# FunAudioLLM/CosyVoice

Measured on NVIDIA H100. Metric: audio-sec/s, CosyVoice2-0.5B zero-shot batch-32, NFE=10, higher is better.
Workload: dtype bf16

## Files before the change

### cosyvoice_b200/csrc/api.cu

```cuda
#include "common.cuh"
#include <string.h>
#include <algorithm>

void hift_build(cvk_ctx* ctx);
void hift_f0(cvk_ctx* ctx, const float* mel, const int* lens, int B, float* f0_out, cudaStream_t st);
void hift_source(cvk_ctx* ctx, const float* f0, const int* lens, int B, const float* noise, float* source_out, cudaStream_t st);
void hift_decode(cvk_ctx* ctx, const float* mel, const int* lens, int B, const float* source, float* wav, cudaStream_t st);
void hift_inference(cvk_ctx* ctx, const float* mel, const int* lens, int B, const float* noise, const float* cache_source,
                    const int* cache_lens, float* wav, float* source_out, cudaStream_t st);
void flow_build(cvk_ctx* ctx, const int* cfg, int ncfg);
void flow_encoder(cvk_ctx* ctx, const int32_t* tokens, const int* lens, int B, int streaming, int context_len, float* h, cudaStream_t st);
void flow_estimator(cvk_ctx* ctx, const float* x, const float* mu, const float* t, const float* spks, const float* cond, const int* lens,
                    int B, int streaming, float* out, cudaStream_t st);
void flow_cfm_solve(cvk_ctx* ctx, const float* mu, const float* spks, const float* cond, const int* lens, int B, const float* z,
                    int n_timesteps, float cfg_rate, int streaming, float* out, cudaStream_t st);
void flow_inference(cvk_ctx* ctx, const int32_t* tokens, const int* token_lens, const float* prompt_feat, const int* prompt_feat_lens,
                    const float* embedding, int B, int n_timesteps, int streaming, int finalize, float* mel, cudaStream_t st);
void flow_set_noise(cvk_ctx* ctx, const float* noise_tm, int T, int on_device);
void llm_build(cvk_ctx* ctx, const int* cfg, int ncfg);
cvk_lm_session* llm_session_create(cvk_ctx* ctx, int max_batch, int max_context);
void llm_session_destroy(cvk_ctx* ctx, cvk_lm_session* s);
void hift3_build(cvk_ctx* ctx);
void hift3_set_noise(cvk_ctx* ctx, const float* rand_ini, const float* sine_noise, long long n, int on_device);
void hift3_inference(cvk_ctx* ctx, const float* mel, const int* lens, const int* finalize, int B, float* wav, float* f0_out,
// ... 22 lines not shown
                    const float* uniforms, const int32_t* ignore_eos, int32_t* out_ids, cudaStream_t st);
void llm_decode_attention_op(cvk_ctx* ctx, const float* partial, int splits, int rows, const float* bias, float* k_cache, float* v_cache,
                             const int* ctx_len_host, int max_ctx, float* out, cudaStream_t st);
void llm_decode_layers_op(cvk_ctx* ctx, int B, const int* ctx_len_host, int max_ctx, float* x, float* k_cache, float* v_cache,
                          float* xn_out, float* att_out, float* ffa_out, cudaStream_t st);
void llm_sample_step_op(cvk_ctx* ctx, float* logits, int B, int V, const float* uniforms, const int32_t* min_len, const int32_t* max_len,
                        int32_t* out_ids, int out_ld, int32_t* out_count, int32_t* done, int* ctx_len, const int* base_len, int* live,
                        const float* speech_emb, float* next_x, const float* gamma, float* xn, cudaStream_t st);
void llm_log_softmax_op(cvk_ctx* ctx, float* x, int rows, int V, cudaStream_t st);
void mel_spectrogram(cvk_ctx* ctx, const float* wav, const int* lens, int B, int fmax_hz, float* mel, cudaStream_t st);
void mel_init(cvk_ctx* ctx);
void mel_resample(cvk_ctx* ctx, const float* mel, const int* lens, const int* out_lens, int B, float* out, cudaStream_t st);
void prompt_feat_init(cvk_ctx* ctx);

#define CVK_API_BEGIN            \
  if (!ctx) return CVK_ERR_INVALID; \
  try {                          \
    cudaSetDevice(ctx->device);
#define CVK_API_END                                  \
    return CVK_OK;                                   \
  } catch (const CvkError& e) {                      \
    ctx->last_error = e.what();                      \
    return e.code;                                   \
  } catch (const std::exception& e) {                \
    ctx->last_error = std::string("internal: ") + e.what(); \
    return CVK_ERR_INVALID;                          \
  }

typedef CUresult (*EncodeTiledFn)(CUtensorMap*, CUtensorMapDataType, cuuint32_t, void*, const cuuint64_t*, const cuuint64_t*,
                                  const cuuint32_t*, const cuuint32_t*, CUtensorMapInterleave, CUtensorMapSwizzle,
                                  CUtensorMapL2promotion, CUtensorMapFloatOOBfill);

void encode_tma_map(cvk_ctx* ctx, CUtensorMap* map, const void* base, int rank, const cuuint64_t* dims, const cuuint64_t* strides,
                    const cuuint32_t* box, int dtype, CUtensorMapL2promotion l2, const char* what) {
  CVK_REQUIRE(rank == 2 || rank == 3, std::string("tensor map ") + what + ": rank 2 or 3");
  const cuuint32_t es[3] = {1, 1, 1};
  CUresult r = ((EncodeTiledFn)ctx->encode_tiled)(map, dtype == DT_F32 ? CU_TENSOR_MAP_DATA_TYPE_FLOAT32 : CU_TENSOR_MAP_DATA_TYPE_BFLOAT16, rank,
                                                  const_cast<void*>(base), dims, strides, box, es, CU_TENSOR_MAP_INTERLEAVE_NONE,
                                                  CU_TENSOR_MAP_SWIZZLE_128B, l2, CU_TENSOR_MAP_FLOAT_OOB_FILL_NONE);
  CVK_REQUIRE(r == CUDA_SUCCESS, std::string("cuTensorMapEncodeTiled(") + what + ") failed: " + std::to_string((int)r));
}

extern "C" {

const char* cvk_version(void) { return "libcvk 0.1 (sm_90a)"; }

int cvk_create(int device, int precision, size_t workspace_bytes, cvk_ctx** out) {
  if (!out) return CVK_ERR_INVALID;
  *out = nullptr;
  int n = 0;
  if (cudaGetDeviceCount(&n) != cudaSuccess || n <= device || device < 0) return CVK_ERR_CUDA;
  if (precision != CVK_PREC_FP32 && precision != CVK_PREC_BF16) return CVK_ERR_INVALID;
  if (cudaSetDevice(device) != cudaSuccess) return CVK_ERR_CUDA;
  cudaDeviceProp prop;
  if (cudaGetDeviceProperties(&prop, device) != cudaSuccess) return CVK_ERR_CUDA;
  if (prop.major != 9) return CVK_ERR_CUDA;
  void* encode = nullptr;
  cudaDriverEntryPointQueryResult qres;
  if (cudaGetDriverEntryPoint("cuTensorMapEncodeTiled", &encode, cudaEnableDefault, &qres) != cudaSuccess ||
      qres != cudaDriverEntryPointSuccess || !encode)
    return CVK_ERR_CUDA;
  try {
    gemm_tc_setup();
    attention_tc_setup();
    skinny_setup();
    hift3_setup();
  } catch (const std::exception&) {
    return CVK_ERR_CUDA;
  }
  cvk_ctx* ctx = new cvk_ctx();
  ctx->device = device;
  ctx->precision = precision;
// ... 22 lines not shown
  delete ctx;
}

const char* cvk_last_error(cvk_ctx* ctx) { return ctx ? ctx->last_error.c_str() : "null context"; }
thread_local int cvk_in_capture = 0;
int64_t cvk_launch_count(cvk_ctx* ctx) { return ctx ? ctx->launches.load() : 0; }
int cvk_stream_create(cvk_ctx* ctx, void** out) {
  CVK_API_BEGIN
  CVK_REQUIRE(out != nullptr, "cvk_stream_create: bad arguments");
  cudaStream_t s = nullptr;
  CVK_CHECK_CUDA(cudaStreamCreateWithFlags(&s, cudaStreamNonBlocking));
  *out = (void*)s;
  CVK_API_END
}
void cvk_stream_destroy(cvk_ctx* ctx, void* stream) {
  if (!ctx || !stream) return;
  cudaSetDevice(ctx->device);
  cudaStreamDestroy((cudaStream_t)stream);
}
double cvk_last_op_ms(cvk_ctx* ctx) { return ctx ? ctx->op_ms : 0.0; }
int cvk_debug_read(cvk_ctx* ctx, long long* out, int n) {
  if (!ctx || !ctx->tl || !out || n != 4096) return CVK_ERR_INVALID;
  cudaSetDevice(ctx->device);
  if (cudaMemcpy(out, ctx->tl, 4096 * sizeof(long long), cudaMemcpyDeviceToHost) != cudaSuccess) return CVK_ERR_CUDA;
  return CVK_OK;
}

int cvk_set_option(cvk_ctx* ctx, const char* key, int value) {
  CVK_API_BEGIN
  std::string k(key ? key : "");
  if (k == "use_tc") ctx->use_tc = value;
  else if (k == "flow_fused_ff") ctx->flow_fused_ff = value;
  else if (k == "flow_qkv_panel") ctx->flow_qkv_panel = value;
  else if (k == "tc_epi") ctx->tc_epi = value;
  else if (k == "tc_persist") ctx->tc_persist = value;
  else if (k == "op_out_bf16") ctx->op_out_bf16 = value;
  else if (k == "op_iters") ctx->op_iters = value;
  else if (k == "use_graph") ctx->use_graph = value;
  else if (k == "use_tc_attn") ctx->use_tc_attn = value;
  else if (k == "use_skinny") ctx->use_skinny = value;
  else if (k == "lm_fused") ctx->lm_fused = value;
  else if (k == "pdl") ctx->pdl = value;
  else if (k == "lm_mega") ctx->lm_mega = value;
  else if (k == "enc_tc_attn") ctx->enc_tc_attn = value;
  else if (k == "hift_f16") ctx->hift_f16 = value;
  else if (k == "mega_coop") ctx->mega_coop = value;
  else if (k == "chain_timeline") {
    if (value && !ctx->tl) {
      ctx->tl = ctx->dmalloc(4096 * sizeof(long long));
      CVK_CHECK_CUDA(cudaMemset(ctx->tl, 0, 4096 * sizeof(long long)));
    }
    if (!value) ctx->tl = nullptr;
  }
  else throw CvkError(CVK_ERR_INVALID, "unknown option: " + k);
  CVK_API_END
}

int cvk_profile(cvk_ctx* ctx, int enable) {
  CVK_API_BEGIN
  CVK_CHECK_CUDA(cudaDeviceSynchronize());
  for (auto& r : ctx->prof) { ctx->event_pool.push_back(r.a); ctx->event_pool.push_back(r.b); }
  ctx->prof.clear();
  ctx->prof_on = enable;
  CVK_API_END
}

// ... 697 lines not shown
```

### cosyvoice_b200/csrc/cvk_internal.h

```cpp
#pragma once
#include <cuda_runtime.h>
#include <cuda_bf16.h>
#include <cuda_fp16.h>
#include <cuda.h>
#include <stdint.h>
#include <stdio.h>
#include <string>
#include <vector>
#include <map>
#include <unordered_map>
#include <stdexcept>
#include <atomic>

#include "../../include/cvk.h"

typedef __nv_bfloat16 bf16;

struct CvkError : std::runtime_error {
  int code;
  CvkError(int c, const std::string& m) : std::runtime_error(m), code(c) {}
};

#define CVK_CHECK_CUDA(expr)                                                                       \
  do {                                                                                             \
// ... 124 lines not shown
  void* prompt_feat_model = nullptr;
  void* encode_tiled = nullptr;
  std::atomic<int64_t> launches{0};
  int op_out_bf16 = 0;
  int op_iters = 0;
  double op_ms = 0.0;
  int tc_epi = 2;
  int tc_persist = 2;
  void* tl = nullptr;
  int tl_seq = 0;
  long long* tl_next() {
    if (!tl) return nullptr;
    long long* p = (long long*)tl + 4 * (tl_seq % 1024);
    ++tl_seq;
    return p;
  }
  int prof_on = 0;
  std::vector<ProfRec> prof;
  std::unordered_map<const void*, void*> tiled;
  std::vector<cudaEvent_t> event_pool;
  int pdl = 1;
  int lm_fused = 1;
  int hift_f16 = 1;
  int build_f16 = 0;
  int enc_tc_attn = 1;
  int lm_mega = 0;
  int mega_coop = 1;
  int use_skinny = 1;
  int use_tc_attn = 1;
  int use_graph = 1;
  int use_tc = 1;
  int flow_fused_ff = 1;
  int flow_qkv_panel = 1;

  void* dmalloc(size_t bytes) {
    void* p = nullptr;
    CVK_CHECK_CUDA(cudaMalloc(&p, bytes ? bytes : 16));
    owned.push_back(p);
    return p;
  }
  const RawTensor& get_raw(const std::string& name) const {
    auto it = raw.find(name);
    if (it == raw.end()) throw CvkError(CVK_ERR_MISSING_WEIGHT, "missing weight tensor: " + name);
    return it->second;
  }
  bool has_raw(const std::string& name) const { return raw.find(name) != raw.end(); }
};

template <typename... KArgs, typename... Args>
inline void launch_ex(void (*kern)(KArgs...), dim3 grid, dim3 block, size_t smem, cudaStream_t st, bool pdl, Args&&... args) {
  cudaLaunchConfig_t cfg = {};
  cfg.gridDim = grid;
  cfg.blockDim = block;
  cfg.dynamicSmemBytes = smem;
  cfg.stream = st;
  cudaLaunchAttribute at[1];
  if (pdl) {
    at[0].id = cudaLaunchAttributeProgrammaticStreamSerialization;
    at[0].val.programmaticStreamSerializationAllowed = 1;
    cfg.attrs = at;
    cfg.numAttrs = 1;
  }
  CVK_CHECK_CUDA(cudaLaunchKernelEx(&cfg, kern, KArgs(std::forward<Args>(args))...));
}

void encode_tma_map(cvk_ctx* ctx, CUtensorMap* map, const void* base, int rank, const cuuint64_t* dims, const cuuint64_t* strides,
                    const cuuint32_t* box, int dtype, CUtensorMapL2promotion l2, const char* what);
void gemm_tc_setup();
void attention_tc_setup();
void skinny_setup();
void hift3_setup();

Seqs make_seqs(cvk_ctx* ctx, const int* lens, int B, int gap, int scale, int extra_front, cudaStream_t st, bool with_row2seq = true);
Seqs scale_seqs(cvk_ctx* ctx, const Seqs& s, int scale, int extra_front, cudaStream_t st, bool with_row2seq = true);

ConvW make_linear(cvk_ctx* ctx, const std::string& wname, const std::string& bname);
ConvW make_conv(cvk_ctx* ctx, const float* w_oik , const float* bias, int N, int K, int taps,
                int dil, int shift0);
ConvW make_conv_named(cvk_ctx* ctx, const std::string& wname, const std::string& bname, int dil, int shift0);
float* fold_weight_norm(cvk_ctx* ctx, const std::string& prefix, int64_t* numel_out);
void finish_convw(cvk_ctx* ctx, ConvW& w);
float* dev_copy_f32(cvk_ctx* ctx, const float* src_dev, size_t n);

void conv_gemm(cvk_ctx* ctx, cudaStream_t st, const Mat& A, const ConvW& W, const Epilogue& ep);
void conv_gemm_simt(cvk_ctx* ctx, cudaStream_t st, const Mat& A, const ConvW& W, const Epilogue& ep);
void conv_gemm_tc(cvk_ctx* ctx, cudaStream_t st, const Mat& A, const ConvW& W, const Epilogue& ep);
void ffn_fused(cvk_ctx* ctx, cudaStream_t st, const Mat& x, const int* row2seq, const float* ln3_g, const float* ln3_b, const ConvW& w1,
               const ConvW& w2, const float* ln_g, const float* ln_b, const Mat& out);
void flow_ff(cvk_ctx* ctx, cudaStream_t st, const Mat& x, const int* row2seq, const float* ln3_g, const float* ln3_b, const ConvW& ff1,
             const ConvW& ff2, const float* ln_g, const float* ln_b, const Mat& out, const Mat& xn, const Mat& hid);
size_t skinny_scratch_floats(int rows, int maxN);
const bf16* skinny_tiled_weights(cvk_ctx* ctx, const ConvW& W);
int conv_gemm_skinny_ex(cvk_ctx* ctx, cudaStream_t st, const Mat& A, const ConvW& W, const Epilogue& ep, float* scratch, size_t scratch_floats,
                        int mode);
void conv_gemm_skinny(cvk_ctx* ctx, cudaStream_t st, const Mat& A, const ConvW& W, const Epilogue& ep, float* scratch, size_t scratch_floats);

void zero_mat(cvk_ctx* ctx, cudaStream_t st, const Mat& m);
void layernorm(cvk_ctx* ctx, cudaStream_t st, const Mat& x, const float* gamma, const float* beta, float eps, int act,
               float post_scale, const int* row2seq, const Mat& out, const float* rowvec = nullptr, int rowvec_ld = 0);
void unpack_rows_skip(cvk_ctx* ctx, cudaStream_t st, const Mat& in, const Seqs& s, const int* skip_host, float* dense, int C);
Seqs shrink_seqs(cvk_ctx* ctx, const Seqs& s, int drop_tail, cudaStream_t st);
Seqs shrink_seqs(cvk_ctx* ctx, const Seqs& s, const int* drop_tail_host , cudaStream_t st);
Seqs subseqs(cvk_ctx* ctx, const Seqs& s, const int* skip_host, cudaStream_t st);
void rmsnorm(cvk_ctx* ctx, cudaStream_t st, const Mat& x, const float* gamma, float eps, const Mat& out);
void act_copy(cvk_ctx* ctx, cudaStream_t st, const Mat& x, int act, float param, const float* alpha, const int* row2seq,
              const Mat& out);
void act_copy_scaled(cvk_ctx* ctx, cudaStream_t st, const Mat& x, float pre_scale, int act, float param, const float* alpha,
                     const int* row2seq, const Mat& out);
void pack_rows(cvk_ctx* ctx, cudaStream_t st, const float* dense, int C, const Seqs& s, const Mat& out);
void unpack_rows(cvk_ctx* ctx, cudaStream_t st, const Mat& in, const Seqs& s, int skip, float* dense, int C);
void bcast_rows(cvk_ctx* ctx, cudaStream_t st, const float* vec, int C, int vec_ld, const Seqs& s, const Mat& out);
void convert_mat(cvk_ctx* ctx, cudaStream_t st, const Mat& in, const Mat& out);

struct KvGeom {
  const int* d_kstart = nullptr;
  const int* d_klen = nullptr;
  const int* d_qoff = nullptr;
};
void whisper_log_mel(cvk_ctx* ctx, const float* wav, const int* lens, int B, float* out, cudaStream_t st);
void kaldi_fbank80(cvk_ctx* ctx, const float* wav, const int* lens, int B, int subtract_mean, float* out, cudaStream_t st);
struct cvk_flow_stream;
// ... 46 lines not shown
```

### cosyvoice_b200/csrc/gemm_tc.cu

```cuda
#include "common.cuh"
#include "wgmma.cuh"
#include "tma.cuh"

namespace {

constexpr int TC_BM = 128;
constexpr int TC_BK = 64;
constexpr int TC_THREADS = 384;

__device__ __forceinline__ void epi_store16(const EpiDev& e, int r, int n0, int N, const float* acc) {
  if (n0 + 16 > N) {
    for (int i = 0; i < 16 && n0 + i < N; ++i) epi_store<true>(e, r, n0 + i, acc[i]);
    return;
  }
  int seq = 0;
  bool valid = true;
  if (e.row2seq) {
    seq = e.row2seq[r];
    valid = seq >= 0;
  }
  float v[16];
#pragma unroll
  for (int i = 0; i < 16; ++i) v[i] = acc[i];
  if (e.bias) {
// ... 156 lines not shown
    const float* rv = e.rowvec + (size_t)seq * e.rowvec_ld + n0;
#pragma unroll
    for (int i = 0; i < 16; i += 4) {
      const float4 b = *reinterpret_cast<const float4*>(rv + i);
      v[i] += b.x; v[i + 1] += b.y; v[i + 2] += b.z; v[i + 3] += b.w;
    }
  }
  act16_fast(e.act1, v, e.act1_param, e.alpha1 ? e.alpha1 + n0 : nullptr);
#pragma unroll
  for (int i = 0; i < 16; ++i) v[i] *= e.scale;
  if (e.resid && rin) {
    const float* rp = e.resid + (size_t)r * e.resid_ld + n0;
#pragma unroll
    for (int i = 0; i < 16; i += 4) {
      const float4 b = *reinterpret_cast<const float4*>(rp + i);
      v[i] += b.x; v[i + 1] += b.y; v[i + 2] += b.z; v[i + 3] += b.w;
    }
  }
  if (!valid) {
#pragma unroll
    for (int i = 0; i < 16; ++i) v[i] = 0.f;
  }
  if (e.out2) {
#pragma unroll
    for (int i = 0; i < 16; ++i) w2[i] = v[i];
    act16_fast(e.act2, w2, e.act2_param, e.alpha2 ? e.alpha2 + n0 : nullptr);
    if (!valid) {
#pragma unroll
      for (int i = 0; i < 16; ++i) w2[i] = 0.f;
    }
  }
}

__device__ __forceinline__ void stage_store16(uint32_t stg, int dtype, int row, int c, const float* v) {
  if (dtype != DT_F32) {
    const uint32_t sub = stg + (uint32_t)(c >> 6) * 16384u + (uint32_t)row * 128u;
    const uint32_t ch = (uint32_t)((c & 63) >> 3);
    uint32_t pk[8];
    if (dtype == DT_BF16) {
#pragma unroll
      for (int i = 0; i < 16; i += 2) {
        __nv_bfloat162 h2 = __floats2bfloat162_rn(v[i], v[i + 1]);
        pk[i >> 1] = *reinterpret_cast<uint32_t*>(&h2);
      }
    } else {
#pragma unroll
      for (int i = 0; i < 16; i += 2) pk[i >> 1] = (uint32_t)f32_to_16(v[i], DT_F16) | ((uint32_t)f32_to_16(v[i + 1], DT_F16) << 16);
    }
    asm volatile("st.shared.v4.b32 [%0], {%1,%2,%3,%4};" ::"r"(sub + ((ch ^ (uint32_t)(row & 7)) << 4)), "r"(pk[0]), "r"(pk[1]), "r"(pk[2]), "r"(pk[3]) : "memory");
    asm volatile("st.shared.v4.b32 [%0], {%1,%2,%3,%4};" ::"r"(sub + (((ch + 1) ^ (uint32_t)(row & 7)) << 4)), "r"(pk[4]), "r"(pk[5]), "r"(pk[6]), "r"(pk[7]) : "memory");
  } else {
    const uint32_t sub = stg + (uint32_t)(c >> 5) * 16384u + (uint32_t)row * 128u;
    const uint32_t ch = (uint32_t)((c & 31) >> 2);
#pragma unroll
    for (int j = 0; j < 4; ++j) {
      asm volatile("st.shared.v4.b32 [%0], {%1,%2,%3,%4};" ::"r"(sub + (((ch + j) ^ (uint32_t)(row & 7)) << 4)), "r"(__float_as_uint(v[4 * j])),
                   "r"(__float_as_uint(v[4 * j + 1])), "r"(__float_as_uint(v[4 * j + 2])), "r"(__float_as_uint(v[4 * j + 3]))
                   : "memory");
    }
  }
}

constexpr uint32_t TC_STG_BYTES = 65536;

template <int BN, int NSTG>
__global__ void __launch_bounds__(TC_THREADS, 1)
conv_gemm_wg_kernel(const __grid_constant__ CUtensorMap tmap_a, const __grid_constant__ CUtensorMap tmap_w,
                    const __grid_constant__ CUtensorMap tmap_o, const __grid_constant__ CUtensorMap tmap_o2, int N, int K, int taps,
                    int dil, int shift0, int rowsOut, EpiDev ep, int epi_mode, int ntn, int ntiles) {
  extern __shared__ uint8_t smem_raw[];
  __shared__ __align__(8) uint64_t bar_full[NSTG];
  __shared__ __align__(8) uint64_t bar_empty[NSTG];
  __shared__ __align__(16) float s_bias[BN];
  constexpr uint32_t A_BYTES = TC_BM * TC_BK * 2;
  constexpr uint32_t B_BYTES = BN * TC_BK * 2;
  constexpr uint32_t STAGE_BYTES = A_BYTES + B_BYTES;
  const uint32_t smem_base = (smem_u32(smem_raw) + 1023u) & ~1023u;
  const uint32_t stg_base = smem_base + NSTG * STAGE_BYTES;
  const int warp = threadIdx.x >> 5, lane = threadIdx.x & 31;
  const int kchunks = (K + TC_BK - 1) / TC_BK;
  const int iters = taps * kchunks;

  if (threadIdx.x == 0) {
    for (int s = 0; s < NSTG; ++s) {
      mbar_init(smem_u32(&bar_full[s]), 1);
      mbar_init(smem_u32(&bar_empty[s]), 8);
    }
    asm volatile("fence.mbarrier_init.release.cluster;" ::: "memory");
  }
  __syncthreads();

  if (warp < 4) {
    if (warp == 0 && lane == 0) {
// ... 421 lines not shown
    const int rb = wg * 64 + (warp & 3) * 16 + (lane >> 2);
#pragma unroll
    for (int j = 0; j < 32; ++j) {
      const int col = 8 * j + 2 * q;
      const float2 b = *reinterpret_cast<const float2*>(p.b2 + col);
      *reinterpret_cast<float2*>(stg + rb * FF_OLD + col) = make_float2(o[4 * j] + b.x, o[4 * j + 1] + b.y);
      *reinterpret_cast<float2*>(stg + (rb + 8) * FF_OLD + col) = make_float2(o[4 * j + 2] + b.x, o[4 * j + 3] + b.y);
    }
  }
  asm volatile("bar.sync 1, 256;" ::: "memory");

  for (int i = 0; i < 16; ++i) {
    const int row = cw * 16 + i, r = r0 + row;
    if (r >= p.rows) break;
    const bool valid = p.row2seq[r] >= 0;
    float* xp = p.x + (size_t)r * p.ldx;
    const float* sp = stg + row * FF_OLD;
    const float4 sa = *reinterpret_cast<const float4*>(sp + c0), sb = *reinterpret_cast<const float4*>(sp + c1);
    const float4 xa = *reinterpret_cast<const float4*>(xp + c0), xb = *reinterpret_cast<const float4*>(xp + c1);
    float v[8] = {sa.x + xa.x, sa.y + xa.y, sa.z + xa.z, sa.w + xa.w, sb.x + xb.x, sb.y + xb.y, sb.z + xb.z, sb.w + xb.w};
    if (!valid) {
#pragma unroll
      for (int j = 0; j < 8; ++j) v[j] = 0.f;
    }
    *reinterpret_cast<float4*>(xp + c0) = make_float4(v[0], v[1], v[2], v[3]);
    *reinterpret_cast<float4*>(xp + c1) = make_float4(v[4], v[5], v[6], v[7]);
    if (p.ln_g && valid) ln256_warp(v, p.ln_g, p.ln_b, 1e-5f, c0, c1);
    bf16* op = p.out + (size_t)r * p.ldo;
    __nv_bfloat162 h0 = __floats2bfloat162_rn(v[0], v[1]), h1 = __floats2bfloat162_rn(v[2], v[3]);
    __nv_bfloat162 h2 = __floats2bfloat162_rn(v[4], v[5]), h3 = __floats2bfloat162_rn(v[6], v[7]);
    *reinterpret_cast<uint2*>(op + c0) = make_uint2(*reinterpret_cast<uint32_t*>(&h0), *reinterpret_cast<uint32_t*>(&h1));
    *reinterpret_cast<uint2*>(op + c1) = make_uint2(*reinterpret_cast<uint32_t*>(&h2), *reinterpret_cast<uint32_t*>(&h3));
  }
}

}

void conv_gemm_tc(cvk_ctx* ctx, cudaStream_t st, const Mat& A, const ConvW& W, const Epilogue& ep) {
  CVK_REQUIRE((A.dtype == DT_BF16 && W.w16 != nullptr) || (A.dtype == DT_F16 && W.wf16 != nullptr), "conv_gemm_tc: 16-bit operands (A and W of the same kind) required");
  const void* w16p = A.dtype == DT_F16 ? (const void*)W.wf16 : (const void*)W.w16;
  CVK_REQUIRE(A.cols >= W.K, "conv_gemm_tc: A has fewer columns than K");
  CVK_REQUIRE(W.K % 8 == 0 && A.ld % 8 == 0 && ((uintptr_t)A.p & 15) == 0, "conv_gemm_tc: operands must be 16-byte aligned");
  CVK_REQUIRE(ep.out.p != nullptr && ep.out.cols >= W.N, "conv_gemm_tc: bad output");
  const int BN = W.N > 64 ? 128 : 64;
  CUtensorMap ta, tw;
  {
    const cuuint64_t dims[2] = {(cuuint64_t)W.K, (cuuint64_t)A.rows};
    const cuuint64_t strides[1] = {(cuuint64_t)A.ld * 2};
    const cuuint32_t box[2] = {TC_BK, TC_BM};
    encode_tma_map(ctx, &ta, A.p, 2, dims, strides, box, A.dtype, CU_TENSOR_MAP_L2_PROMOTION_L2_128B, "A");
  }
  {
    const cuuint64_t dims[3] = {(cuuint64_t)W.K, (cuuint64_t)W.taps, (cuuint64_t)W.N};
    const cuuint64_t strides[2] = {(cuuint64_t)W.K * 2, (cuuint64_t)W.K * W.taps * 2};
    const cuuint32_t box[3] = {TC_BK, 1, (cuuint32_t)BN};
    encode_tma_map(ctx, &tw, w16p, 3, dims, strides, box, A.dtype, CU_TENSOR_MAP_L2_PROMOTION_L2_256B, "W");
  }
  EpiDev e = to_dev(ep);
  e.ab_f16 = A.dtype == DT_F16;
  if (!e.bias) e.bias = W.bias;
  int rowsOut = ep.out.rows;
  CVK_REQUIRE((ep.out.ld * ep.out.esize()) % 16 == 0 && ((uintptr_t)ep.out.p & 15) == 0, "conv_gemm_tc: output rows must be 16-byte aligned");
  CVK_REQUIRE(!ep.resid.p || (ep.resid.ld % 4 == 0 && ((uintptr_t)ep.resid.p & 15) == 0), "conv_gemm_tc: residual alignment");
  CVK_REQUIRE(!(ep.resid.p && ep.rowvec), "conv_gemm_tc: residual and per-sequence vector cannot be combined");
  CVK_REQUIRE(!ep.rowvec || (ep.rowvec_ld % 4 == 0 && ((uintptr_t)ep.rowvec & 15) == 0), "conv_gemm_tc: rowvec alignment");
  CVK_REQUIRE(!ep.out2.p || ((ep.out2.ld * ep.out2.esize()) % 16 == 0 && ((uintptr_t)ep.out2.p & 15) == 0), "conv_gemm_tc: out2 alignment");
// ... 27 lines not shown
}

void ffn_fused(cvk_ctx* ctx, cudaStream_t st, const Mat& x, const int* row2seq, const float* ln3_g, const float* ln3_b, const ConvW& w1,
               const ConvW& w2, const float* ln_g, const float* ln_b, const Mat& out) {
  CVK_REQUIRE(x.dtype == DT_F32 && x.cols == FF_C && x.ld % 4 == 0 && ((uintptr_t)x.p & 15) == 0, "ffn_fused: x must be fp32 [rows, 256], 16-byte aligned rows");
  CVK_REQUIRE(out.dtype == DT_BF16 && out.cols == FF_C && out.rows >= x.rows && out.ld % 8 == 0 && ((uintptr_t)out.p & 15) == 0,
              "ffn_fused: out must be bf16 [rows, 256], 16-byte aligned rows");
  CVK_REQUIRE(w1.N == FF_HID && w1.K == FF_C && w1.taps == 1 && w1.w16 && w1.bias && w2.N == FF_C && w2.K == FF_HID && w2.taps == 1 && w2.w16 &&
                  w2.bias && row2seq && ln3_g && ln3_b && (!ln_g || ln_b),
              "ffn_fused: unexpected weights");
  CVK_REQUIRE((((uintptr_t)ln3_g | (uintptr_t)ln3_b | (uintptr_t)ln_g | (uintptr_t)ln_b | (uintptr_t)w1.bias | (uintptr_t)w2.bias) & 15) == 0,
              "ffn_fused: LayerNorm and bias vectors must be 16-byte aligned");
  CUtensorMap t1, t2;
  auto mk = [&](CUtensorMap* m, const bf16* w, int N, int K, int box_n) {
    const cuuint64_t dims[2] = {(cuuint64_t)K, (cuuint64_t)N};
    const cuuint64_t strides[1] = {(cuuint64_t)K * 2};
    const cuuint32_t box[2] = {64, (cuuint32_t)box_n};
    encode_tma_map(ctx, m, w, 2, dims, strides, box, DT_BF16, CU_TENSOR_MAP_L2_PROMOTION_L2_256B, "ffn weights");
  };
  mk(&t1, w1.w16, FF_HID, FF_C, FF_HC);
  mk(&t2, w2.w16, FF_C, FF_HID, FF_C);
  FfnDev p;
  p.x = x.f32(); p.ldx = x.ld; p.rows = x.rows; p.row2seq = row2seq;
  p.ln3_g = ln3_g; p.ln3_b = ln3_b; p.b1 = w1.bias; p.b2 = w2.bias; p.ln_g = ln_g; p.ln_b = ln_b;
  p.out = out.b16(); p.ldo = out.ld;
  const double flops = 4.0 * x.rows * (double)FF_C * FF_HID;
  const double bytes = (double)x.rows * FF_C * (4 + 4 + 2) + 2.0 * FF_C * FF_HID * 2;
  ProfScope ps(ctx, st, FAM_GEMM_TC, flops, bytes);
  ffn_fused_kernel<<<ceil_div(x.rows, TC_BM), TC_THREADS, FF_SMEM, st>>>(t1, t2, p);
  ctx->launches++;
  CVK_LAUNCH_CHECK();
}

void gemm_tc_setup() {
  CVK_CHECK_CUDA(cudaFuncSetAttribute(conv_gemm_wg_kernel<128, 4>, cudaFuncAttributeMaxDynamicSharedMemorySize, (int)wg_smem<128, 4>()));
  CVK_CHECK_CUDA(cudaFuncSetAttribute(conv_gemm_wg_kernel<64, 4>, cudaFuncAttributeMaxDynamicSharedMemorySize, (int)wg_smem<64, 4>()));
  CVK_CHECK_CUDA(cudaFuncSetAttribute(qkv_panel_kernel, cudaFuncAttributeMaxDynamicSharedMemorySize, (int)QP_SMEM));
  CVK_CHECK_CUDA(cudaFuncSetAttribute(ffn_fused_kernel, cudaFuncAttributeMaxDynamicSharedMemorySize, (int)FF_SMEM));
}
```

### cosyvoice_b200/csrc/hift.cu

```cuda
#include "common.cuh"

namespace {

constexpr int kUps[3] = {8, 5, 3};
constexpr int kUpK[3] = {16, 11, 7};
constexpr int kRbK[3] = {3, 7, 11};
constexpr int kSrcRbK[3] = {7, 7, 11};
constexpr int kDil[3] = {1, 3, 5};
constexpr int kCh[4] = {512, 256, 128, 64};
constexpr int kUpscale = 480;
constexpr int kStftLd = 24;

struct ResBlockW {
  ConvW c1[3], c2[3];
  float* a1[3];
  float* a2[3];
};

}

struct HiftModel {
  bool half_weights = false;
  ConvW f0_conv[5];
  ConvW f0_cls;
// ... 336 lines not shown

static int* upload_ints(cvk_ctx* ctx, const std::vector<int>& v, cudaStream_t st) {
  int* d = (int*)ctx->arena.alloc(sizeof(int) * v.size());
  CVK_CHECK_CUDA(cudaMemcpyAsync(d, v.data(), sizeof(int) * v.size(), cudaMemcpyHostToDevice, st));
  return d;
}

static std::vector<int> prefix_offsets(const int* lens, int B) {
  std::vector<int> off(B);
  int acc = 0;
  for (int b = 0; b < B; ++b) { off[b] = acc; acc += lens[b]; }
  return off;
}

static void hift_source_packed(cvk_ctx* ctx, cudaStream_t st, const Seqs& s0, const int* lens, const Mat& f0, const float* noise,
                               float* src_packed) {
  HiftModel* m = ctx->hift;
  float* phase = (float*)ctx->arena.alloc(sizeof(float) * 9 * (size_t)s0.R);
  phase_kernel<<<s0.B, 32, 0, st>>>(f0.f32(), f0.ld, s0.d_start, s0.d_len, phase);
  ctx->launches++;
  CVK_LAUNCH_CHECK();
  CVK_CHECK_CUDA(cudaMemsetAsync(src_packed, 0, sizeof(float) * (size_t)s0.R * kUpscale, st));
  int* noff = upload_ints(ctx, prefix_offsets(lens, s0.B), st);
  int bx = ceil_div(s0.max_len * kUpscale, 256);
  if (bx > 512) bx = 512;
  source_kernel<<<dim3(bx, s0.B), 256, 0, st>>>(f0.f32(), f0.ld, phase, s0.d_start, s0.d_len, noise, noff, m->src_w, m->src_b, src_packed);
  ctx->launches++;
  CVK_LAUNCH_CHECK();
}

static void run_resblock(cvk_ctx* ctx, cudaStream_t st, const ResBlockW& rb, const Seqs& s, const Mat& x ,
                         const Mat& a , const Mat& ya, const Mat& xr ,
                         const Mat& final_out, int final_accumulate) {
  for (int d = 0; d < 3; ++d) {
    Epilogue e1;
    e1.act1 = ACT_SNAKE;
    e1.alpha1 = rb.a2[d];
    e1.row2seq = s.d_row2seq;
    e1.out = ya;
    conv_gemm(ctx, st, a, rb.c1[d], e1);
    Epilogue e2;
    e2.resid = d == 0 ? x : xr;
    e2.row2seq = s.d_row2seq;
    if (d < 2) {
      e2.out = xr;
      e2.act2 = ACT_SNAKE;
      e2.alpha2 = rb.a1[d + 1];
      e2.out2 = a;
    } else {
      e2.out = final_out;
      e2.accumulate = final_accumulate;
    }
    conv_gemm(ctx, st, ya, rb.c2[d], e2);
  }
}

static Mat hift_body(cvk_ctx* ctx, cudaStream_t st, const HiftGeom& g, const Mat& mel32, const float* src_packed,
                     const HiftModel* m = nullptr, const int* d_len_sig = nullptr) {
  if (!m) m = ctx->hift;
  const int adt = (ctx->act_dtype == DT_BF16 && m->half_weights) ? DT_F16 : ctx->act_dtype;
  const Seqs& s0 = g.s0;
  const Seqs& s3 = g.lv[2];
  Mat stft = arena_mat(ctx, adt, s3.R, kStftLd, kStftLd);
  zero_mat(ctx, st, stft);
  {
    int F = s0.max_len * 120 + 1;
    int bx = ceil_div(F, 128);
    if (bx > 1024) bx = 1024;
    if (adt == DT_F32) stft16_kernel<float><<<dim3(bx, s0.B), 128, 0, st>>>(src_packed, s0.d_start, s0.d_len, s3.d_start, stft.f32(), stft.ld, d_len_sig);
    else if (adt == DT_F16) stft16_kernel<__half><<<dim3(bx, s0.B), 128, 0, st>>>(src_packed, s0.d_start, s0.d_len, s3.d_start, (__half*)stft.p, stft.ld, d_len_sig);
    else stft16_kernel<bf16><<<dim3(bx, s0.B), 128, 0, st>>>(src_packed, s0.d_start, s0.d_len, s3.d_start, stft.b16(), stft.ld, d_len_sig);
    ctx->launches++;
    CVK_LAUNCH_CHECK();
  }
  Mat mel_a = mel32;
  if (adt != DT_F32) {
    mel_a = arena_mat(ctx, adt, s0.R, 80);
    convert_mat(ctx, st, mel32, mel_a);
  }
  Mat xin = arena_mat(ctx, adt, s0.R, 512);
  {
    Epilogue e;
    e.act1 = ACT_LRELU;
    e.act1_param = 0.1f;
    e.row2seq = s0.d_row2seq;
    e.out = xin;
// ... 562 lines not shown
```

### cosyvoice_b200/csrc/wgmma.cuh

```cuda
#pragma once
#include <cstdint>

__device__ __forceinline__ uint64_t wg_desc_sw128(uint32_t saddr) {
  return (uint64_t)((saddr & 0x3FFFFu) >> 4) | (1ull << 16) | (64ull << 32) | (1ull << 62);
}
__device__ __forceinline__ void wg_fence() { asm volatile("wgmma.fence.sync.aligned;" ::: "memory"); }
__device__ __forceinline__ void wg_commit() { asm volatile("wgmma.commit_group.sync.aligned;" ::: "memory"); }
template <int N> __device__ __forceinline__ void wg_wait() { asm volatile("wgmma.wait_group.sync.aligned %0;" ::"n"(N) : "memory"); }
template <int R> __device__ __forceinline__ void wg_touch(float* d) {
#pragma unroll
  for (int i = 0; i < R; ++i) asm volatile("" : "+f"(d[i])::"memory");
}

template <int N, int F16> __device__ __forceinline__ void wgmma_ss(float* d, uint64_t a, uint64_t b, int acc);

template <> __device__ __forceinline__ void wgmma_ss<32, 0>(float* d, uint64_t a, uint64_t b, int acc) {
  asm volatile(
      "{\n\t.reg .pred p;\n\tsetp.ne.b32 p, %18, 0;\n\t"
      "wgmma.mma_async.sync.aligned.m64n32k16.f32.bf16.bf16 {%0,%1,%2,%3,%4,%5,%6,%7,%8,%9,%10,%11,%12,%13,%14,%15}, %16, %17, p, 1, 1, 0, 0;\n\t}"
      : "+f"(d[0]), "+f"(d[1]), "+f"(d[2]), "+f"(d[3]), "+f"(d[4]), "+f"(d[5]), "+f"(d[6]), "+f"(d[7]), "+f"(d[8]), "+f"(d[9]), "+f"(d[10]), "+f"(d[11]), "+f"(d[12]), "+f"(d[13]), "+f"(d[14]), "+f"(d[15])
      : "l"(a), "l"(b), "r"(acc));
}

template <> __device__ __forceinline__ void wgmma_ss<32, 1>(float* d, uint64_t a, uint64_t b, int acc) {
  asm volatile(
      "{\n\t.reg .pred p;\n\tsetp.ne.b32 p, %18, 0;\n\t"
      "wgmma.mma_async.sync.aligned.m64n32k16.f32.f16.f16 {%0,%1,%2,%3,%4,%5,%6,%7,%8,%9,%10,%11,%12,%13,%14,%15}, %16, %17, p, 1, 1, 0, 0;\n\t}"
      : "+f"(d[0]), "+f"(d[1]), "+f"(d[2]), "+f"(d[3]), "+f"(d[4]), "+f"(d[5]), "+f"(d[6]), "+f"(d[7]), "+f"(d[8]), "+f"(d[9]), "+f"(d[10]), "+f"(d[11]), "+f"(d[12]), "+f"(d[13]), "+f"(d[14]), "+f"(d[15])
      : "l"(a), "l"(b), "r"(acc));
}

template <> __device__ __forceinline__ void wgmma_ss<64, 0>(float* d, uint64_t a, uint64_t b, int acc) {
  asm volatile(
      "{\n\t.reg .pred p;\n\tsetp.ne.b32 p, %34, 0;\n\t"
      "wgmma.mma_async.sync.aligned.m64n64k16.f32.bf16.bf16 {%0,%1,%2,%3,%4,%5,%6,%7,%8,%9,%10,%11,%12,%13,%14,%15,%16,%17,%18,%19,%20,%21,%22,%23,%24,%25,%26,%27,%28,%29,%30,%31}, %32, %33, p, 1, 1, 0, 0;\n\t}"
      : "+f"(d[0]), "+f"(d[1]), "+f"(d[2]), "+f"(d[3]), "+f"(d[4]), "+f"(d[5]), "+f"(d[6]), "+f"(d[7]), "+f"(d[8]), "+f"(d[9]), "+f"(d[10]), "+f"(d[11]), "+f"(d[12]), "+f"(d[13]), "+f"(d[14]), "+f"(d[15]), "+f"(d[16]), "+f"(d[17]), "+f"(d[18]), "+f"(d[19]), "+f"(d[20]), "+f"(d[21]), "+f"(d[22]), "+f"(d[23]), "+f"(d[24]), "+f"(d[25]), "+f"(d[26]), "+f"(d[27]), "+f"(d[28]), "+f"(d[29]), "+f"(d[30]), "+f"(d[31])
      : "l"(a), "l"(b), "r"(acc));
// ... 65 lines not shown
```

Baseline: 433.5.

## Fuse HiFT resblock conv pair into one warp-specialized wgmma kernel

Adds a resblock_step kernel that runs the dilated conv c1 with its snake epilogue, keeps the intermediate activation in shared memory in an interleaved layout, then runs conv c2 with its residual and snake epilogue in the same CTA. A TMA producer warp streams the input tile and the weights of both convs. This replaces two conv_gemm launches per dilation step and removes the global round trip of the ya intermediate. In exchange, the kernel recomputes halo rows because each tile produces only BM minus (taps2 minus 1) outputs, and it ping-pongs the a buffer, which adds shared memory pressure and lowers occupancy.

```diff
diff --git a/cosyvoice_b200/csrc/api.cu b/cosyvoice_b200/csrc/api.cu
--- a/cosyvoice_b200/csrc/api.cu
+++ b/cosyvoice_b200/csrc/api.cu
@@ -78,12 +78,12 @@
                                   CUtensorMapL2promotion, CUtensorMapFloatOOBfill);
 
 void encode_tma_map(cvk_ctx* ctx, CUtensorMap* map, const void* base, int rank, const cuuint64_t* dims, const cuuint64_t* strides,
-                    const cuuint32_t* box, int dtype, CUtensorMapL2promotion l2, const char* what) {
+                    const cuuint32_t* box, int dtype, CUtensorMapL2promotion l2, const char* what, CUtensorMapSwizzle swizzle) {
   CVK_REQUIRE(rank == 2 || rank == 3, std::string("tensor map ") + what + ": rank 2 or 3");
   const cuuint32_t es[3] = {1, 1, 1};
   CUresult r = ((EncodeTiledFn)ctx->encode_tiled)(map, dtype == DT_F32 ? CU_TENSOR_MAP_DATA_TYPE_FLOAT32 : CU_TENSOR_MAP_DATA_TYPE_BFLOAT16, rank,
                                                   const_cast<void*>(base), dims, strides, box, es, CU_TENSOR_MAP_INTERLEAVE_NONE,
-                                                  CU_TENSOR_MAP_SWIZZLE_128B, l2, CU_TENSOR_MAP_FLOAT_OOB_FILL_NONE);
+                                                  swizzle, l2, CU_TENSOR_MAP_FLOAT_OOB_FILL_NONE);
   CVK_REQUIRE(r == CUDA_SUCCESS, std::string("cuTensorMapEncodeTiled(") + what + ") failed: " + std::to_string((int)r));
 }
 
@@ -172,6 +172,7 @@
   if (k == "use_tc") ctx->use_tc = value;
   else if (k == "flow_fused_ff") ctx->flow_fused_ff = value;
   else if (k == "flow_qkv_panel") ctx->flow_qkv_panel = value;
+  else if (k == "hift_fused_rb") ctx->hift_fused_rb = value;
   else if (k == "tc_epi") ctx->tc_epi = value;
   else if (k == "tc_persist") ctx->tc_persist = value;
   else if (k == "op_out_bf16") ctx->op_out_bf16 = value;
diff --git a/cosyvoice_b200/csrc/cvk_internal.h b/cosyvoice_b200/csrc/cvk_internal.h
--- a/cosyvoice_b200/csrc/cvk_internal.h
+++ b/cosyvoice_b200/csrc/cvk_internal.h
@@ -180,6 +180,7 @@
   int use_tc = 1;
   int flow_fused_ff = 1;
   int flow_qkv_panel = 1;
+  int hift_fused_rb = 1;
 
   void* dmalloc(size_t bytes) {
     void* p = nullptr;
@@ -213,7 +214,8 @@
 }
 
 void encode_tma_map(cvk_ctx* ctx, CUtensorMap* map, const void* base, int rank, const cuuint64_t* dims, const cuuint64_t* strides,
-                    const cuuint32_t* box, int dtype, CUtensorMapL2promotion l2, const char* what);
+                    const cuuint32_t* box, int dtype, CUtensorMapL2promotion l2, const char* what,
+                    CUtensorMapSwizzle swizzle = CU_TENSOR_MAP_SWIZZLE_128B);
 void gemm_tc_setup();
 void attention_tc_setup();
 void skinny_setup();
@@ -235,6 +237,7 @@
 void conv_gemm_tc(cvk_ctx* ctx, cudaStream_t st, const Mat& A, const ConvW& W, const Epilogue& ep);
 void ffn_fused(cvk_ctx* ctx, cudaStream_t st, const Mat& x, const int* row2seq, const float* ln3_g, const float* ln3_b, const ConvW& w1,
                const ConvW& w2, const float* ln_g, const float* ln_b, const Mat& out);
+void resblock_step_tc(cvk_ctx* ctx, cudaStream_t st, const Mat& a, const ConvW& c1, const Epilogue& ep1, const ConvW& c2, const Epilogue& ep2);
 void flow_ff(cvk_ctx* ctx, cudaStream_t st, const Mat& x, const int* row2seq, const float* ln3_g, const float* ln3_b, const ConvW& ff1,
              const ConvW& ff2, const float* ln_g, const float* ln_b, const Mat& out, const Mat& xn, const Mat& hid);
 size_t skinny_scratch_floats(int rows, int maxN);
diff --git a/cosyvoice_b200/csrc/gemm_tc.cu b/cosyvoice_b200/csrc/gemm_tc.cu
--- a/cosyvoice_b200/csrc/gemm_tc.cu
+++ b/cosyvoice_b200/csrc/gemm_tc.cu
@@ -212,21 +212,25 @@
   }
 }
 
+__device__ __forceinline__ void pack16(int dtype, const float* v, uint32_t* pk) {
+  if (dtype == DT_BF16) {
+#pragma unroll
+    for (int i = 0; i < 16; i += 2) {
+      __nv_bfloat162 h2 = __floats2bfloat162_rn(v[i], v[i + 1]);
+      pk[i >> 1] = *reinterpret_cast<uint32_t*>(&h2);
+    }
+  } else {
+#pragma unroll
+    for (int i = 0; i < 16; i += 2) pk[i >> 1] = (uint32_t)f32_to_16(v[i], DT_F16) | ((uint32_t)f32_to_16(v[i + 1], DT_F16) << 16);
+  }
+}
+
 __device__ __forceinline__ void stage_store16(uint32_t stg, int dtype, int row, int c, const float* v) {
   if (dtype != DT_F32) {
     const uint32_t sub = stg + (uint32_t)(c >> 6) * 16384u + (uint32_t)row * 128u;
     const uint32_t ch = (uint32_t)((c & 63) >> 3);
     uint32_t pk[8];
-    if (dtype == DT_BF16) {
-#pragma unroll
-      for (int i = 0; i < 16; i += 2) {
-        __nv_bfloat162 h2 = __floats2bfloat162_rn(v[i], v[i + 1]);
-        pk[i >> 1] = *reinterpret_cast<uint32_t*>(&h2);
-      }
-    } else {
-#pragma unroll
-      for (int i = 0; i < 16; i += 2) pk[i >> 1] = (uint32_t)f32_to_16(v[i], DT_F16) | ((uint32_t)f32_to_16(v[i + 1], DT_F16) << 16);
-    }
+    pack16(dtype, v, pk);
     asm volatile("st.shared.v4.b32 [%0], {%1,%2,%3,%4};" ::"r"(sub + ((ch ^ (uint32_t)(row & 7)) << 4)), "r"(pk[0]), "r"(pk[1]), "r"(pk[2]), "r"(pk[3]) : "memory");
     asm volatile("st.shared.v4.b32 [%0], {%1,%2,%3,%4};" ::"r"(sub + (((ch + 1) ^ (uint32_t)(row & 7)) << 4)), "r"(pk[4]), "r"(pk[5]), "r"(pk[6]), "r"(pk[7]) : "memory");
   } else {
@@ -239,6 +243,16 @@
                    : "memory");
     }
   }
+}
+
+__device__ __forceinline__ void prefetch_l2(const void* p) { asm volatile("prefetch.global.L2 [%0];" ::"l"(p)); }
+
+__device__ __forceinline__ void interleave_store16(uint32_t tile, uint32_t ld, int dtype, int row, int c, const float* v) {
+  uint32_t pk[8];
+  pack16(dtype, v, pk);
+  const uint32_t p = tile + (uint32_t)(c >> 3) * ld + (uint32_t)row * 16u;
+  asm volatile("st.shared.v4.b32 [%0], {%1,%2,%3,%4};" ::"r"(p), "r"(pk[0]), "r"(pk[1]), "r"(pk[2]), "r"(pk[3]) : "memory");
+  asm volatile("st.shared.v4.b32 [%0], {%1,%2,%3,%4};" ::"r"(p + ld), "r"(pk[4]), "r"(pk[5]), "r"(pk[6]), "r"(pk[7]) : "memory");
 }
 
 constexpr uint32_t TC_STG_BYTES = 65536;
@@ -726,6 +740,185 @@
     *reinterpret_cast<uint2*>(op + c0) = make_uint2(*reinterpret_cast<uint32_t*>(&h0), *reinterpret_cast<uint32_t*>(&h1));
     *reinterpret_cast<uint2*>(op + c1) = make_uint2(*reinterpret_cast<uint32_t*>(&h2), *reinterpret_cast<uint32_t*>(&h3));
   }
+}
+
+constexpr int RS_THREADS = 288;
+constexpr int RS_PAD = 16;
+constexpr int RS_AROWS = 192;
+template <int C> struct RsTile {
+  static constexpr int KC = C / TC_BK;
+  static constexpr int NSTG = 4;
+  static constexpr int CTAS = C == 64 ? 2 : 1;
+  static constexpr uint32_t A_LD = RS_AROWS * 16;
+  static constexpr uint32_t A_BYTES = (C / 8) * A_LD;
+  static constexpr uint32_t B_BYTES = C * TC_BK * 2;
+  static constexpr uint32_t Y_LD = (TC_BM + RS_PAD) * 16;
+  static constexpr uint32_t Y_BYTES = (C / 8) * Y_LD;
+  static constexpr size_t SMEM = (size_t)2 * A_BYTES + (size_t)NSTG * B_BYTES + Y_BYTES + 1024;
+  static_assert(SMEM <= 227 * 1024, "resblock_step_kernel: shared memory");
+};
+
+template <int C>
+__global__ void __launch_bounds__(RS_THREADS, RsTile<C>::CTAS)
+resblock_step_kernel(const __grid_constant__ CUtensorMap tmap_a, const __grid_constant__ CUtensorMap tmap_w1,
+                     const __grid_constant__ CUtensorMap tmap_w2, int taps1, int dil1, int shift1, int taps2, int shift2, int arows,
+                     int rows, int ntiles, EpiDev e1, EpiDev e2) {
+  using T = RsTile<C>;
+  extern __shared__ uint8_t smem_raw[];
+  __shared__ __align__(8) uint64_t bar_full[T::NSTG];
+  __shared__ __align__(8) uint64_t bar_empty[T::NSTG];
+  __shared__ __align__(8) uint64_t bar_afull[2];
+  __shared__ __align__(8) uint64_t bar_aempty[2];
+  __shared__ __align__(16) float s_bias[C];
+  __shared__ __align__(16) float s_vec[3][C];
+  const uint32_t smem_base = (smem_u32(smem_raw) + 1023u) & ~1023u;
+  const uint32_t ring = smem_base + 2 * T::A_BYTES;
+  const uint32_t ya = ring + T::NSTG * T::B_BYTES;
+  const int warp = threadIdx.x >> 5, lane = threadIdx.x & 31;
+  const int ot = TC_BM - (taps2 - 1);
+  const int it1 = taps1 * T::KC, it2 = taps2 * T::KC;
+
+  if (threadIdx.x == 0) {
+    for (int s = 0; s < T::NSTG; ++s) {
+      mbar_init(smem_u32(&bar_full[s]), 1);
+      mbar_init(smem_u32(&bar_empty[s]), 8);
+    }
+    for (int b = 0; b < 2; ++b) {
+      mbar_init(smem_u32(&bar_afull[b]), 1);
+      mbar_init(smem_u32(&bar_aempty[b]), 8);
+    }
+    asm volatile("fence.mbarrier_init.release.cluster;" ::: "memory");
+  }
+  __syncthreads();
+
+  if (warp == 8) {
+    if (lane == 0) {
+      uint32_t it = 0, ti = 0;
+      for (int tile = blockIdx.x; tile < ntiles; tile += gridDim.x, ++ti) {
+        const int y0 = tile * ot + shift2;
+        {
+          const uint32_t b = ti & 1u;
+          mbar_wait(smem_u32(&bar_aempty[b]), ((ti >> 1) & 1u) ^ 1u);
+          const uint32_t fa = smem_u32(&bar_afull[b]);
+          mbar_expect_tx(fa, (uint32_t)(C / 8) * (uint32_t)arows * 16u);
+#pragma unroll
+          for (int g = 0; g < C / 8; ++g) tma_load_2d(smem_base + b * T::A_BYTES + g * T::A_LD, &tmap_a, fa, g * 8, y0 + shift1);
+        }
+        for (int i = 0; i < it1 + it2; ++i, ++it) {
+          const uint32_t s = it % T::NSTG, round = it / T::NSTG;
+          mbar_wait(smem_u32(&bar_empty[s]), (round & 1u) ^ 1u);
+          const uint32_t fb = smem_u32(&bar_full[s]);
+          mbar_expect_tx(fb, T::B_BYTES);
+          const bool first = i < it1;
+          const int ii = first ? i : i - it1;
+          const int j = ii / T::KC, kc = ii - j * T::KC;
+          tma_load_3d(ring + s * T::B_BYTES, first ? &tmap_w1 : &tmap_w2, fb, kc * TC_BK, j, 0);
+        }
+      }
+    }
+    return;
+  }
+  const int ct = threadIdx.x;
+  const int wg = ct >> 7;
+  const int q = lane & 3;
+  const int row = wg * 64 + (warp & 3) * 16 + (lane >> 2) + 8 * (q & 1);
+  const int cq = 16 * (q >> 1);
+  for (int i = ct; i < C; i += 256) {
+    s_bias[i] = e1.bias ? e1.bias[i] : 0.f;
+    s_vec[0][i] = e1.alpha1 ? e1.alpha1[i] : 0.f;
+    s_vec[1][i] = e2.bias ? e2.bias[i] : 0.f;
+    s_vec[2][i] = e2.alpha2 ? e2.alpha2[i] : 0.f;
+  }
+  if (e1.alpha1) e1.alpha1 = s_vec[0];
+  if (e2.bias) e2.bias = s_vec[1];
+  if (e2.alpha2) e2.alpha2 = s_vec[2];
+  for (uint32_t o = (uint32_t)ct * 16u; o < T::Y_BYTES; o += 256u * 16u)
+    asm volatile("st.shared.v4.b32 [%0], {%1,%1,%1,%1};" ::"r"(ya + o), "r"(0) : "memory");
+  asm volatile("bar.sync 1, 256;" ::: "memory");
+
+  float acc[C / 2];
+  auto mma_loop = [&](uint32_t& it, int iters, uint32_t tile_a, uint32_t lda, int row0, int dil) {
+#pragma unroll
+    for (int i = 0; i < C / 2; ++i) acc[i] = 0.f;
+    for (int i = 0; i < iters; ++i, ++it) {
+      const uint32_t s = it % T::NSTG, round = it / T::NSTG;
+      const int j = i / T::KC, kc = i - j * T::KC;
+      const uint32_t a0 = tile_a + (uint32_t)(kc * 8) * lda + (uint32_t)(row0 + j * dil) * 16u;
+      const uint64_t db = wg_desc_sw128(ring + s * T::B_BYTES);
+      uint64_t da[TC_BK / 16];
+#pragma unroll
+      for (int k = 0; k < TC_BK / 16; ++k) da[k] = wg_desc_interleave(a0 + 2 * k * lda, lda, 128);
+      mbar_wait(smem_u32(&bar_full[s]), round & 1u);
+      wg_fence();
+      if (e1.ab_f16) {
+#pragma unroll
+        for (int k = 0; k < TC_BK / 16; ++k) wgmma_ss<C, 1>(acc, da[k], db + (uint64_t)(2 * k), 1);
+      } else {
+#pragma unroll
+        for (int k = 0; k < TC_BK / 16; ++k) wgmma_ss<C, 0>(acc, da[k], db + (uint64_t)(2 * k), 1);
+      }
+      wg_commit();
+      wg_wait<1>();
+      __syncwarp();
+      if (i > 0 && lane == 0) mbar_arrive(smem_u32(&bar_empty[(it - 1) % T::NSTG]));
+    }
+    wg_wait<0>();
+    wg_touch<C / 2>(acc);
+    __syncwarp();
+    if (iters > 0 && lane == 0) mbar_arrive(smem_u32(&bar_empty[(it - 1) % T::NSTG]));
+  };
+
+  uint32_t it = 0, ti = 0;
+  for (int tile = blockIdx.x; tile < ntiles; tile += gridDim.x, ++ti) {
+    const int r0 = tile * ot;
+    const int r = r0 + row;
+    const bool store = row < ot && r < rows;
+    if (C == 64 && store) {
+#pragma unroll
+      for (int cb = 0; cb < C; cb += 32) {
+        if (e2.resid) prefetch_l2(e2.resid + (size_t)r * e2.resid_ld + cb + cq);
+        if (e2.accumulate) prefetch_l2((const float*)e2.out + (size_t)r * e2.out_ld + cb + cq);
+      }
+    }
+    const int yr = r0 + shift2 + row;
+    const bool yin = yr >= 0 && yr < rows;
+    int seq = 0;
+    if (yin && e1.row2seq) seq = e1.row2seq[yr];
+    const bool yvalid = yin && (!e1.row2seq || seq >= 0);
+
+    const uint32_t b = ti & 1u;
+    mbar_wait(smem_u32(&bar_afull[b]), (ti >> 1) & 1u);
+    mma_loop(it, it1, smem_base + b * T::A_BYTES, T::A_LD, wg * 64, dil1);
+    if (lane == 0) mbar_arrive(smem_u32(&bar_aempty[b]));
+    asm volatile("bar.sync 1, 256;" ::: "memory");
+#pragma unroll
+    for (int cb = 0; cb < C; cb += 32) {
+      float a16[16], v[16], w2[16];
+      wg_frag_rows16(acc + cb / 2, lane, a16);
+      const int c = cb + cq;
+      epi_math16p(e1, yr, yin, seq, yvalid, s_bias, c, c, a16, v, w2);
+      interleave_store16(ya, T::Y_LD, e1.out_dtype, row, c, v);
+    }
+    asm volatile("fence.proxy.async.shared::cta;" ::: "memory");
+    asm volatile("bar.sync 1, 256;" ::: "memory");
+
+    mma_loop(it, it2, ya, T::Y_LD, wg * 64, 1);
+#pragma unroll
+    for (int cb = 0; cb < C; cb += 32) {
+      float a16[16];
+      wg_frag_rows16(acc + cb / 2, lane, a16);
+      if (store) epi_store16(e2, r, cb + cq, C, a16);
+    }
+  }
+}
+
+template <int C>
+void launch_resblock_step(cvk_ctx* ctx, cudaStream_t st, const CUtensorMap& ta, const CUtensorMap& tw1, const CUtensorMap& tw2,
+                          const ConvW& c1, const ConvW& c2, int arows, int rows, const EpiDev& e1, const EpiDev& e2) {
+  const int ntiles = ceil_div(rows, TC_BM - (c2.taps - 1));
+  const int grid = std::min(ntiles, RsTile<C>::CTAS * ctx->num_sms);
+  resblock_step_kernel<C><<<grid, RS_THREADS, RsTile<C>::SMEM, st>>>(ta, tw1, tw2, c1.taps, c1.dil, c1.shift0, c2.taps, c2.shift0, arows,
+                                                                     rows, ntiles, e1, e2);
 }
 
 }
@@ -819,7 +1012,56 @@
   CVK_LAUNCH_CHECK();
 }
 
+void resblock_step_tc(cvk_ctx* ctx, cudaStream_t st, const Mat& a, const ConvW& c1, const Epilogue& ep1, const ConvW& c2, const Epilogue& ep2) {
+  const int C = a.cols;
+  CVK_REQUIRE((C == 128 || C == 64) && c1.K == C && c1.N == C && c2.K == C && c2.N == C && c2.dil == 1 && c2.taps <= RS_PAD + 1,
+              "resblock_step: C = 128 or 64 channels, c2 undilated with at most 17 taps");
+  CVK_REQUIRE(a.dtype == DT_F16 || a.dtype == DT_BF16, "resblock_step: 16-bit operand");
+  const void* w1 = a.dtype == DT_F16 ? (const void*)c1.wf16 : (const void*)c1.w16;
+  const void* w2 = a.dtype == DT_F16 ? (const void*)c2.wf16 : (const void*)c2.w16;
+  CVK_REQUIRE(w1 && w2, "resblock_step: no 16-bit weights of the operand's kind");
+  CVK_REQUIRE(a.ld % 8 == 0 && ((uintptr_t)a.p & 15) == 0, "resblock_step: operand rows must be 16-byte aligned");
+  CVK_REQUIRE(!ep1.resid.p && !ep1.rowvec && !ep1.out2.p && !ep1.accumulate, "resblock_step: c1 epilogue is bias, activation and row mask");
+  CVK_REQUIRE(!ep2.rowvec && ep2.out.p && ep2.out.rows == a.rows && ep2.out.cols >= C, "resblock_step: bad output");
+  CVK_REQUIRE((ep2.out.ld * ep2.out.esize()) % 16 == 0 && ((uintptr_t)ep2.out.p & 15) == 0, "resblock_step: output rows must be 16-byte aligned");
+  CVK_REQUIRE(!ep2.resid.p || (ep2.resid.ld % 4 == 0 && ((uintptr_t)ep2.resid.p & 15) == 0), "resblock_step: residual alignment");
+  CVK_REQUIRE(!ep2.out2.p || ((ep2.out2.ld * ep2.out2.esize()) % 16 == 0 && ((uintptr_t)ep2.out2.p & 15) == 0), "resblock_step: out2 alignment");
+  const int arows = TC_BM + (c1.taps - 1) * c1.dil;
+  CVK_REQUIRE(arows <= RS_AROWS, "resblock_step: c1 reaches too far");
+  CUtensorMap ta, tw1, tw2;
+  {
+    const cuuint64_t dims[2] = {(cuuint64_t)C, (cuuint64_t)a.rows};
+    const cuuint64_t strides[1] = {(cuuint64_t)a.ld * 2};
+    const cuuint32_t box[2] = {8, (cuuint32_t)arows};
+    encode_tma_map(ctx, &ta, a.p, 2, dims, strides, box, a.dtype, CU_TENSOR_MAP_L2_PROMOTION_L2_128B, "A", CU_TENSOR_MAP_SWIZZLE_NONE);
+  }
+  auto mkw = [&](CUtensorMap* m, const void* w, const ConvW& W) {
+    const cuuint64_t dims[3] = {(cuuint64_t)C, (cuuint64_t)W.taps, (cuuint64_t)C};
+    const cuuint64_t strides[2] = {(cuuint64_t)C * 2, (cuuint64_t)C * W.taps * 2};
+    const cuuint32_t box[3] = {TC_BK, 1, (cuuint32_t)C};
+    encode_tma_map(ctx, m, w, 3, dims, strides, box, a.dtype, CU_TENSOR_MAP_L2_PROMOTION_L2_256B, "W");
+  };
+  mkw(&tw1, w1, c1);
+  mkw(&tw2, w2, c2);
+  EpiDev e1 = to_dev(ep1), e2 = to_dev(ep2);
+  e1.ab_f16 = e2.ab_f16 = a.dtype == DT_F16;
+  if (!e1.bias) e1.bias = c1.bias;
+  if (!e2.bias) e2.bias = c2.bias;
+  e1.out = nullptr;
+  e1.out_dtype = a.dtype;
+  const double flops = 2.0 * a.rows * (double)C * C * (c1.taps + c2.taps);
+  const double bytes = (double)a.rows * C * (2 + (ep2.resid.p ? 4 : 0) + ep2.out.esize() * (ep2.accumulate ? 2 : 1) + (ep2.out2.p ? ep2.out2.esize() : 0));
+  ProfScope ps(ctx, st, FAM_GEMM_TC, flops, bytes);
+  if (C == 128) launch_resblock_step<128>(ctx, st, ta, tw1, tw2, c1, c2, arows, a.rows, e1, e2);
+  else launch_resblock_step<64>(ctx, st, ta, tw1, tw2, c1, c2, arows, a.rows, e1, e2);
+  ctx->launches++;
+  CVK_LAUNCH_CHECK();
+}
+
 void gemm_tc_setup() {
+  CVK_CHECK_CUDA(cudaFuncSetAttribute(resblock_step_kernel<128>, cudaFuncAttributeMaxDynamicSharedMemorySize, (int)RsTile<128>::SMEM));
+  CVK_CHECK_CUDA(cudaFuncSetAttribute(resblock_step_kernel<64>, cudaFuncAttributeMaxDynamicSharedMemorySize, (int)RsTile<64>::SMEM));
+  CVK_CHECK_CUDA(cudaFuncSetAttribute(resblock_step_kernel<64>, cudaFuncAttributePreferredSharedMemoryCarveout, 100));
   CVK_CHECK_CUDA(cudaFuncSetAttribute(conv_gemm_wg_kernel<128, 4>, cudaFuncAttributeMaxDynamicSharedMemorySize, (int)wg_smem<128, 4>()));
   CVK_CHECK_CUDA(cudaFuncSetAttribute(conv_gemm_wg_kernel<64, 4>, cudaFuncAttributeMaxDynamicSharedMemorySize, (int)wg_smem<64, 4>()));
   CVK_CHECK_CUDA(cudaFuncSetAttribute(qkv_panel_kernel, cudaFuncAttributeMaxDynamicSharedMemorySize, (int)QP_SMEM));
diff --git a/cosyvoice_b200/csrc/hift.cu b/cosyvoice_b200/csrc/hift.cu
--- a/cosyvoice_b200/csrc/hift.cu
+++ b/cosyvoice_b200/csrc/hift.cu
@@ -392,13 +392,14 @@
 static void run_resblock(cvk_ctx* ctx, cudaStream_t st, const ResBlockW& rb, const Seqs& s, const Mat& x ,
                          const Mat& a , const Mat& ya, const Mat& xr ,
                          const Mat& final_out, int final_accumulate) {
+  const bool fused = ctx->hift_fused_rb && ctx->use_tc && a.dtype != DT_F32 && (a.cols == 128 || a.cols == 64);
+  Mat cur = a, nxt = ya;
   for (int d = 0; d < 3; ++d) {
     Epilogue e1;
     e1.act1 = ACT_SNAKE;
     e1.alpha1 = rb.a2[d];
     e1.row2seq = s.d_row2seq;
     e1.out = ya;
-    conv_gemm(ctx, st, a, rb.c1[d], e1);
     Epilogue e2;
     e2.resid = d == 0 ? x : xr;
     e2.row2seq = s.d_row2seq;
@@ -406,12 +407,18 @@
       e2.out = xr;
       e2.act2 = ACT_SNAKE;
       e2.alpha2 = rb.a1[d + 1];
-      e2.out2 = a;
+      e2.out2 = fused ? nxt : a;
     } else {
       e2.out = final_out;
       e2.accumulate = final_accumulate;
     }
-    conv_gemm(ctx, st, ya, rb.c2[d], e2);
+    if (fused) {
+      resblock_step_tc(ctx, st, cur, rb.c1[d], e1, rb.c2[d], e2);
+      std::swap(cur, nxt);
+    } else {
+      conv_gemm(ctx, st, a, rb.c1[d], e1);
+      conv_gemm(ctx, st, ya, rb.c2[d], e2);
+    }
   }
 }
 
diff --git a/cosyvoice_b200/csrc/wgmma.cuh b/cosyvoice_b200/csrc/wgmma.cuh
--- a/cosyvoice_b200/csrc/wgmma.cuh
+++ b/cosyvoice_b200/csrc/wgmma.cuh
@@ -3,6 +3,9 @@
 
 __device__ __forceinline__ uint64_t wg_desc_sw128(uint32_t saddr) {
   return (uint64_t)((saddr & 0x3FFFFu) >> 4) | (1ull << 16) | (64ull << 32) | (1ull << 62);
+}
+__device__ __forceinline__ uint64_t wg_desc_interleave(uint32_t saddr, uint32_t lbo, uint32_t sbo) {
+  return (uint64_t)((saddr & 0x3FFFFu) >> 4) | ((uint64_t)((lbo >> 4) & 0x3FFFu) << 16) | ((uint64_t)((sbo >> 4) & 0x3FFFu) << 32);
 }
 __device__ __forceinline__ void wg_fence() { asm volatile("wgmma.fence.sync.aligned;" ::: "memory"); }
 __device__ __forceinline__ void wg_commit() { asm volatile("wgmma.commit_group.sync.aligned;" ::: "memory"); }
```

After: 436.3, median of 6. No clear change (+0.7%).
